# JeongsooP/RGB-no-more

Hardware: AMD Instinct MI355X
Metric: images/sec JPEG-Ti DCT 512x512 train step (higher is better)
Workload: dtype bf16

## Files before the change

rgb-no-more_amd/csrc/vit.hip:

```cpp
#include "common.h"
#include "../../include/rgbnm.h"

#define TRY(x)                 \
  do {                         \
    int rc__ = (x);            \
    if (rc__ != 0) return rc__; \
  } while (0)

static inline size_t max_sz(size_t a, size_t b) { return a > b ? a : b; }

#include <string.h>
#include <atomic>
#include <mutex>
#include <vector>
#include "internal.h"
namespace {
std::mutex g_trace_mu;
struct TraceRec { hipEvent_t a, b; int tag; double flops, bytes; };
std::vector<TraceRec> g_recs;
std::vector<hipEvent_t> g_event_pool;
hipEvent_t take_event() {
  if (!g_event_pool.empty()) { hipEvent_t e = g_event_pool.back(); g_event_pool.pop_back(); return e; }
  hipEvent_t e = nullptr;
  if (hipEventCreate(&e) != hipSuccess) return nullptr;
  return e;
}
struct Opt { const char* name; std::atomic<int> value; };
Opt g_opts[] = {{"nt_staged", 1}, {"tn_tr", 1}, {"tn_pipe", 1}, {"attn_v2", 1}, {"nt_wres", 1}, {"nt_kpipe", 1}, {"attn_persist", 1}, {"ln_fuse", 1}, {"tn_group", 2}, {"trace", 0}, {"tn_wgs", 512}, {"mlp_fuse", 1}, {"nt_cold", 0}, {"mlp_bwd", 1}, {"nt_small", 1}, {"mlp_dmast", 1}, {"gelu_table", 1}, {"ln_rows", 1}, {"kp8", 1}, {"win_xcd", 1}, {"kp_persist", 1}, {"fwd_chain", 1}, {"bwd_chain", 1}, {"tn_direct", 1}, {"tn_pack", 1}, {"tn_wide", 1}};
}

int rgbnm_trace_begin(int tag, double flops, double bytes, hipStream_t st) {
  int mask = 0;
  for (auto& o : g_opts) if (!strcmp(o.name, "trace")) mask = o.value.load(std::memory_order_relaxed);
  if (!((mask >> tag) & 1)) return -1;
  std::lock_guard<std::mutex> lk(g_trace_mu);
  TraceRec r;
  r.a = take_event();
  r.b = take_event();
  if (!r.a || !r.b) return -1;
  r.tag = tag; r.flops = flops; r.bytes = bytes;
  (void)hipEventRecord(r.a, st);
  g_recs.push_back(r);
  return (int)g_recs.size() - 1;
}
void rgbnm_trace_end(int slot, hipStream_t st) {
  if (slot < 0) return;
  std::lock_guard<std::mutex> lk(g_trace_mu);
  if (slot >= 0 && slot < (int)g_recs.size()) (void)hipEventRecord(g_recs[slot].b, st);
}

extern "C" {

int rgbnm_abi_version(void) { return RGBNM_ABI_VERSION; }

int rgbnm_set_option(const char* name, int value) {
  for (auto& o : g_opts)
    if (name && !strcmp(o.name, name)) { o.value.store(value, std::memory_order_relaxed); return RGBNM_OK; }
  return RGBNM_EINVAL;
}
int rgbnm_get_option(const char* name) {
  for (auto& o : g_opts)
    if (name && !strcmp(o.name, name)) return o.value.load(std::memory_order_relaxed);
  return -1;
}

int rgbnm_trace_reserve(int n_events) {
  if (n_events < 0 || n_events > (1 << 16)) return RGBNM_EINVAL;
  std::lock_guard<std::mutex> lk(g_trace_mu);
  while ((int)g_event_pool.size() < n_events) {
    hipEvent_t e = nullptr;
    if (hipEventCreate(&e) != hipSuccess) return RGBNM_ELAUNCH;
    g_event_pool.push_back(e);
  }
  return RGBNM_OK;
}

int rgbnm_trace_collect(int tag, double* ms_total, double* flops_total, double* bytes_total, int* count) {
  double ms = 0, fl = 0, by = 0;
  int n = 0;
  std::lock_guard<std::mutex> lk(g_trace_mu);
  std::vector<TraceRec> keep;
  for (auto& r : g_recs) {
    if (r.tag != tag) { keep.push_back(r); continue; }
    if (hipEventSynchronize(r.b) != hipSuccess) return RGBNM_ELAUNCH;
    float t = 0.f;
    if (hipEventElapsedTime(&t, r.a, r.b) != hipSuccess) return RGBNM_ELAUNCH;
    ms += t; fl += r.flops; by += r.bytes; ++n;
    g_event_pool.push_back(r.a);
    g_event_pool.push_back(r.b);
  }
  g_recs.swap(keep);
  if (ms_total) *ms_total = ms;
  if (flops_total) *flops_total = fl;
  if (bytes_total) *bytes_total = by;
  if (count) *count = n;
  return RGBNM_OK;
}

const char* rgbnm_strerror(int code) {
  switch (code) {
    case 0: return "ok";
    case RGBNM_EINVAL: return "invalid argument (null pointer, bad shape, alignment or dtype)";
    case RGBNM_ELAUNCH: return "HIP kernel launch failed";
    case RGBNM_EWORKSPACE: return "workspace too small";
    default: return "unknown rgbnm error";
  }
}

static bool fused_dx_lnbwd(int dt, const void* A, int lda, const void* Wt, int ldw, const void* x, const float* gamma,
                           const float* mean, const float* rstd, const void* dres, void* dx, float* dgamma,
                           float* dbeta, int M, int E, int K, void* ws, size_t ws_bytes, hipStream_t st) {
// ... 288 lines not shown
```

rgb-no-more_amd/csrc/vit_chain.hip:

```cpp
#include "common.h"
#include <string.h>
#include <type_traits>
#include "internal.h"
#include "../../include/rgbnm.h"

namespace {

typedef __attribute__((address_space(3))) void* lds_ptr;
typedef const __attribute__((address_space(1))) void* glb_ptr;
typedef unsigned int u32x2 __attribute__((ext_vector_type(2)));
typedef unsigned int u32x4 __attribute__((ext_vector_type(4)));
typedef bf16 bf16x2v __attribute__((ext_vector_type(2)));

constexpr int E = 192, HID = 768, HD = 64, HEADS = 3, NTOK = 196, NTILE = 7, NPAD = 224, INNER = HEADS * HD;
constexpr int NCW = 7, NTHREADS = 64 * (NCW + 1);
constexpr int ROWB = 128;
constexpr int SLOT = 24576;
constexpr int A_SLOT0 = 0;
constexpr int K_OFF = 3 * SLOT;
constexpr int ARR = NPAD * ROWB;
constexpr int V_OFF = K_OFF + ARR;
constexpr int STGA_OFF = V_OFF + ARR;
constexpr int STG_TILE = 32 * ROWB;
constexpr int MISC_OFF = STGA_OFF + 6 * STG_TILE + 4 * ROWB;
// ... 86 lines not shown
  template <typename F> static __device__ __forceinline__ void run(F&&) {}
};

__device__ __forceinline__ bf16x8 pack8(u32x2 lo, u32x2 hi) {
  u32x4 v = {lo[0], lo[1], hi[0], hi[1]};
  return __builtin_bit_cast(bf16x8, v);
}
template <int T>
__device__ __forceinline__ void tfrag4(unsigned a0, Frag<bf16> (&f)[4]) {
  u32x2 r0, r1, r2, r3, r4, r5, r6, r7;
  const unsigned a00 = a0, a01 = (a0 ^ 32u) + 1024u, a10 = a0 ^ 64u, a11 = (a0 ^ 96u) + 1024u;
  asm volatile(
      "ds_read_b64_tr_b16 %0, %8 offset:%12\n\t"
      "ds_read_b64_tr_b16 %1, %9 offset:%12\n\t"
      "ds_read_b64_tr_b16 %2, %10 offset:%12\n\t"
      "ds_read_b64_tr_b16 %3, %11 offset:%12\n\t"
      "ds_read_b64_tr_b16 %4, %8 offset:%13\n\t"
      "ds_read_b64_tr_b16 %5, %9 offset:%13\n\t"
      "ds_read_b64_tr_b16 %6, %10 offset:%13\n\t"
      "ds_read_b64_tr_b16 %7, %11 offset:%13\n\t"
      "s_waitcnt lgkmcnt(0)"
      : "=&v"(r0), "=&v"(r1), "=&v"(r2), "=&v"(r3), "=&v"(r4), "=&v"(r5), "=&v"(r6), "=&v"(r7)
      : "v"(a00), "v"(a01), "v"(a10), "v"(a11), "i"(T * 4096), "i"(T * 4096 + 2048)
      : "memory");
  __builtin_amdgcn_sched_barrier(0);
  f[0].v = pack8(r0, r1);
  f[1].v = pack8(r2, r3);
  f[2].v = pack8(r4, r5);
  f[3].v = pack8(r6, r7);
}
typedef bf16 bf16x4v __attribute__((ext_vector_type(4)));
typedef __attribute__((address_space(3))) bf16x4v* lds_b64_ptr;
__device__ __forceinline__ u32x2 tr_read(const unsigned char* smem, unsigned off) {
  return __builtin_bit_cast(u32x2, __builtin_amdgcn_ds_read_tr16_b64_v4bf16((lds_b64_ptr)(smem + off)));
}
template <int T>
__device__ __forceinline__ void tfrag4_b(const unsigned char* smem, unsigned a0, Frag<bf16> (&f)[4]) {
  const unsigned a00 = a0, a01 = (a0 ^ 32u) + 1024u, a10 = a0 ^ 64u, a11 = (a0 ^ 96u) + 1024u;
  f[0].v = pack8(tr_read(smem, a00 + T * 4096), tr_read(smem, a01 + T * 4096));
  f[1].v = pack8(tr_read(smem, a10 + T * 4096), tr_read(smem, a11 + T * 4096));
  f[2].v = pack8(tr_read(smem, a00 + T * 4096 + 2048), tr_read(smem, a01 + T * 4096 + 2048));
  f[3].v = pack8(tr_read(smem, a10 + T * 4096 + 2048), tr_read(smem, a11 + T * 4096 + 2048));
}
__device__ __forceinline__ Frag<bf16> pfrag(const float (&p)[16], int fi) {
  Frag<bf16> f;
#pragma unroll
  for (int j = 0; j < 8; ++j) f.v[j] = (bf16)p[fi * 8 + j];
  return f;
}

__device__ __forceinline__ unsigned opaque(unsigned v) {
  asm volatile("" : "+v"(v));
  return v;
}
__device__ __forceinline__ void wg_barrier() {
  asm volatile("" ::: "memory");
  __builtin_amdgcn_s_barrier();
  asm volatile("" ::: "memory");
}
template <int N> __device__ __forceinline__ void wait_vm() { asm volatile("s_waitcnt vmcnt(%0)" ::"n"(N) : "memory"); }
__device__ __forceinline__ void wait_lds() { asm volatile("s_waitcnt lgkmcnt(0)" ::: "memory"); }
#ifndef X_STORE
#define X_STORE 1
#endif
template <typename V, typename P>
__device__ __forceinline__ void gstore(P* ptr, const V& v) {
#if X_STORE == 1
  __builtin_nontemporal_store(v, reinterpret_cast<V*>(ptr));
#elif X_STORE == 2
  asm volatile("global_store_dwordx4 %0, %1, off sc1\n\ts_nop 2" ::"v"(reinterpret_cast<V*>(ptr)), "v"(v) : "memory");
#elif X_STORE == 3
  asm volatile("global_store_dwordx4 %0, %1, off sc0 sc1\n\ts_nop 2" ::"v"(reinterpret_cast<V*>(ptr)), "v"(v) : "memory");
#else
  *reinterpret_cast<V*>(ptr) = v;
#endif
}

#ifdef X_LDSWAIT
__device__ __forceinline__ void own_tile_fence() { wait_lds(); }
#else
__device__ __forceinline__ void own_tile_fence() { asm volatile("" ::: "memory"); }
#endif

template <int NKB>
__device__ __forceinline__ void dma_linear(const unsigned char* src, unsigned char* dst, int lane) {
#pragma unroll
  for (int i = 0; i < NKB; ++i)
    __builtin_amdgcn_global_load_lds((glb_ptr)(src + i * 1024 + lane * 16), (lds_ptr)(dst + i * 1024), 16, 0, 0);
}
__device__ __forceinline__ void dma_f32x192(const float* src, unsigned char* dst, int lane) {
#pragma unroll
  for (int i = 0; i < 3; ++i)
    __builtin_amdgcn_global_load_lds((glb_ptr)(src + 64 * i + lane), (lds_ptr)(dst + 256 * i), 4, 0, 0);
}

struct Rows { u32x4 v[12]; };
__device__ __forceinline__ float bf_lo(unsigned u) { return __builtin_bit_cast(float, u << 16); }
__device__ __forceinline__ float bf_hi(unsigned u) { return __builtin_bit_cast(float, u & 0xffff0000u); }
__device__ __forceinline__ unsigned pack2(float a, float b) {
  const bf16x2v v = {(bf16)a, (bf16)b};
  unsigned r = __builtin_bit_cast(unsigned, v);
  asm volatile("" : "+v"(r));
  return r;
}
__device__ __forceinline__ bf16x8 as_bf16x8(u32x4 v) { return __builtin_bit_cast(bf16x8, v); }

__device__ __forceinline__ void ln_stats(const Rows& x, float& mu, float& rs, float eps) {
  float s0 = 0.f, s1 = 0.f;
#pragma unroll
  for (int c = 0; c < 12; ++c)
#pragma unroll
    for (int d = 0; d < 4; ++d) {
      const unsigned u = opaque(x.v[c][d]);
      s0 += bf_lo(u);
      s1 += bf_hi(u);
    }
  float s = s0 + s1;
  s += __shfl_xor(s, 32, 64);
  mu = s * (1.f / E);
  float q0 = 0.f, q1 = 0.f;
#pragma unroll
  for (int c = 0; c < 12; ++c)
#pragma unroll
    for (int d = 0; d < 4; ++d) {
      const unsigned u = opaque(x.v[c][d]);
      const float d0 = bf_lo(u) - mu, d1 = bf_hi(u) - mu;
      q0 = __builtin_fmaf(d0, d0, q0);
      q1 = __builtin_fmaf(d1, d1, q1);
    }
  float q = q0 + q1;
  q += __shfl_xor(q, 32, 64);
  rs = rsqrtf(__builtin_fmaf(q, 1.f / E, eps));
}
__device__ __forceinline__ void ln_apply(const Rows& x, float mu, float rs, const float* gb, int g, Rows& y) {
#ifdef X_NOLN
#pragma unroll
  for (int c = 0; c < 12; ++c) y.v[c] = x.v[c];
  return;
#endif
#pragma unroll
  for (int c = 0; c < 12; ++c) {
    const float* gp = gb + 16 * c + 8 * g;
    const f32x4 g0 = *reinterpret_cast<const f32x4*>(gp), g1 = *reinterpret_cast<const f32x4*>(gp + 4);
    const f32x4 b0 = *reinterpret_cast<const f32x4*>(gp + E), b1 = *reinterpret_cast<const f32x4*>(gp + E + 4);
#pragma unroll
    for (int d = 0; d < 4; ++d) {
      const float gm0 = d < 2 ? g0[2 * d] : g1[2 * d - 4], gm1 = d < 2 ? g0[2 * d + 1] : g1[2 * d - 3];
      const float bt0 = d < 2 ? b0[2 * d] : b1[2 * d - 4], bt1 = d < 2 ? b0[2 * d + 1] : b1[2 * d - 3];
      const unsigned u = opaque(x.v[c][d]);
      y.v[c][d] = pack2(__builtin_fmaf((bf_lo(u) - mu) * rs, gm0, bt0), __builtin_fmaf((bf_hi(u) - mu) * rs, gm1, bt1));
    }
    if (c & 1) __builtin_amdgcn_sched_barrier(0);
  }
}

__device__ __forceinline__ void tile_out(unsigned char* smem, unsigned stg, const u32x4& p0, const u32x4& p1, const u32x4& p2,
                                         const u32x4& p3, bf16* dst, int ld, int live) {
  const int ln = lane_id_here();
  const unsigned wo = stg + (unsigned)((ln & 31) * ROWB + (((ln >> 5) ^ (ln & 7)) << 4));
  if ((ln & 31) < live) {
    *reinterpret_cast<u32x4*>(smem + wo) = p0;
    *reinterpret_cast<u32x4*>(smem + (wo ^ 32u)) = p1;
    *reinterpret_cast<u32x4*>(smem + (wo ^ 64u)) = p2;
    *reinterpret_cast<u32x4*>(smem + (wo ^ 96u)) = p3;
  }
  own_tile_fence();
  const int rl = ln >> 3, seg = ln & 7;
  const unsigned ro = stg + (unsigned)(rl * ROWB + ((seg ^ rl) << 4));
  bf16* gp = dst + (size_t)rl * ld + seg * 8;
  u32x4 v[4];
#pragma unroll
  for (int i = 0; i < 4; ++i) v[i] = *reinterpret_cast<const u32x4*>(smem + ro + i * 8 * ROWB);
#ifndef X_NOSAVE
  if (live == 32) {
#pragma unroll
    for (int i = 0; i < 4; ++i) gstore(gp + (size_t)i * 8 * ld, v[i]);
  } else {
#pragma unroll
    for (int i = 0; i < 4; ++i)
      if (i * 8 + rl < live) gstore(gp + (size_t)i * 8 * ld, v[i]);
  }
#endif
  own_tile_fence();
}
__device__ __forceinline__ void rows_out(unsigned char* smem, unsigned stg, const Rows& x, bf16* dst, int live) {
#pragma unroll
  for (int t = 0; t < 3; ++t) {
    tile_out(smem, stg, x.v[4 * t], x.v[4 * t + 1], x.v[4 * t + 2], x.v[4 * t + 3], dst + 64 * t, E, live);
    __builtin_amdgcn_sched_barrier(0);
  }
}

__device__ __forceinline__ void gemm_k192(f32x16& acc, const unsigned char* sW, int ht, const Rows& x, const Geo& L) {
  int wbase = L.l31 * (E * 2) + ((L.g ^ L.fl) << 4) + ht * 32 * (E * 2);
  asm volatile("" : "+v"(wbase));
  Frag<bf16> fb;
#pragma unroll
  for (int c = 0; c < 12; ++c) {
    Frag<bf16> fx;
#ifdef X_HALFW
    if ((c & 1) == 0)
#endif
    fb.v = *reinterpret_cast<const bf16x8*>(sW + ((wbase ^ ((c % 4) << 5)) + 128 * (c / 4)));
    fx.v = as_bf16x8(x.v[c]);
    mma(acc, fb, fx);
  }
}

template <int DEPTH>
__device__ __forceinline__ void gemm_k192x2(f32x16& a0, f32x16& a1, const unsigned char* sW, const Rows& x, const Geo& L) {
  int wb0 = L.l31 * (E * 2) + ((L.g ^ L.fl) << 4);
  asm volatile("" : "+v"(wb0));
  const int wb1 = wb0 + 32 * (E * 2);
  Frag<bf16> fb[24];
#pragma unroll
  for (int i = 0; i < 24; ++i) {
    const int c = i >> 1;
    fb[i].v = *reinterpret_cast<const bf16x8*>(sW + ((((i & 1) ? wb1 : wb0) ^ ((c % 4) << 5)) + 128 * (c / 4)));
  }
#pragma unroll
  for (int i = 0; i < 24; ++i) {
    Frag<bf16> fx;
    fx.v = as_bf16x8(x.v[i >> 1]);
    mma((i & 1) ? a1 : a0, fb[i], fx);
  }
  __builtin_amdgcn_sched_group_barrier(0x100, DEPTH, 0);
#pragma unroll
  for (int i = 0; i < 24 - DEPTH; ++i) {
    __builtin_amdgcn_sched_group_barrier(0x008, 1, 0);
    __builtin_amdgcn_sched_group_barrier(0x100, 1, 0);
  }
#pragma unroll
  for (int i = 0; i < DEPTH; ++i) __builtin_amdgcn_sched_group_barrier(0x008, 1, 0);
}

#ifdef CHAIN_PROF
#ifndef CHAIN_PROF_BLK
#define CHAIN_PROF_BLK 1
#endif
__device__ unsigned long long g_chain_prof[8 * 8 * 128];
#define CP(i)                                                                                          \
  do {                                                                                                 \
    if (ib == CHAIN_PROF_BLK && blockIdx.x < 8) {                                                      \
      const unsigned long long t_ = __builtin_amdgcn_s_memtime();                                      \
      if ((threadIdx.x & 63) == 0) g_chain_prof[(blockIdx.x * 8 + (threadIdx.x >> 6)) * 128 + (i)] = t_; \
    }                                                                                                  \
  } while (0)
#define CP_RT(i)                                                                                       \
  do {                                                                                                 \
    if (blockIdx.x < 8 && (threadIdx.x & 63) == 0)                                                     \
      g_chain_prof[(blockIdx.x * 8 + (threadIdx.x >> 6)) * 128 + (i)] = __builtin_amdgcn_s_memrealtime(); \
  } while (0)
#else
#define CP(i) do {} while (0)
#define CP_RT(i) do {} while (0)
#endif
#define BAR(s) do { CP(2 * (s)); wg_barrier(); CP(2 * (s) + 1); } while (0)
// ... 324 lines not shown
          pf = pfrag(pr, 1);
          mma(o[0], vv[2], pf);
          mma(o[1], vv[3], pf);
        });
#else
        {
          Frag<bf16> kc[4], kn[4];
#pragma unroll
          for (int c = 0; c < 4; ++c) kc[c].v = *reinterpret_cast<const bf16x8*>(Ks + (rb ^ (unsigned)(c << 5)));
          __builtin_amdgcn_sched_barrier(0);
          TileLoop<NTILE>::run([&](auto tc) {
            constexpr int t = decltype(tc)::value;
            f32x16 acc;
#pragma unroll
            for (int r = 0; r < 16; ++r) acc[r] = 0.f;
#pragma unroll
            for (int c = 0; c < 4; ++c) mma(acc, kc[c], qf[c]);
            Frag<bf16> vv[4];
            tfrag4_b<t>(smem, vt, vv);
            if (t + 1 < NTILE) {
#pragma unroll
              for (int c = 0; c < 4; ++c)
                kn[c].v = *reinterpret_cast<const bf16x8*>(Ks + (rb ^ (unsigned)(c << 5)) + (t + 1) * 32 * ROWB);
            }
            float pr[16];
#pragma unroll
            for (int r = 0; r < 16; ++r) {
#ifdef X_NOEXP
              pr[r] = fmaf(acc[r], c2, -mc2);
#else
              pr[r] = __builtin_amdgcn_exp2f(fmaf(acc[r], c2, -mc2));
#endif
              if (t * 32 + 32 > NTOK && t * 32 + acc_row(r, L.lane) >= NTOK) pr[r] = 0.f;
              sum += pr[r];
            }
            Frag<bf16> pf = pfrag(pr, 0);
            mma(o[0], vv[0], pf);
            mma(o[1], vv[1], pf);
            pf = pfrag(pr, 1);
            mma(o[0], vv[2], pf);
            mma(o[1], vv[3], pf);
            __builtin_amdgcn_sched_group_barrier(0x008, 4, 0);
            if (t + 1 < NTILE) __builtin_amdgcn_sched_group_barrier(0x100, 12, 0);
            else __builtin_amdgcn_sched_group_barrier(0x100, 8, 0);
            __builtin_amdgcn_sched_group_barrier(0x008, 4, 0);
            __builtin_amdgcn_sched_barrier(0);
#pragma unroll
            for (int c = 0; c < 4; ++c) kc[c] = kn[c];
          });
        }
#endif
        sum += __shfl_xor(sum, 32, 64);
        const float inv = 1.f / sum;
        if (L.g == 0 && L.l31 < live) b.lse[((size_t)img * HEADS + h) * NTOK + row0 + L.l31] = mx * p.scale + __logf(sum);
        u32x4 op[4];
#pragma unroll
        for (int dt = 0; dt < 2; ++dt)
#pragma unroll
          for (int hs = 0; hs < 2; ++hs) {
#pragma unroll
            for (int d = 0; d < 4; ++d) op[2 * dt + hs][d] = pack2(o[dt][8 * hs + 2 * d] * inv, o[dt][8 * hs + 2 * d + 1] * inv);
            of[h][2 * dt + hs].v = as_bf16x8(op[2 * dt + hs]);
          }
        {
          const int ln = lane_id_here();
          const unsigned wo = stg + (unsigned)((ln & 31) * ROWB + ((ln & 7) << 4) + (ln >> 5) * 8);
          if ((ln & 31) < live)
#pragma unroll
          for (int dt = 0; dt < 2; ++dt)
#pragma unroll
            for (int rq = 0; rq < 4; ++rq) {
              const u32x4 src = op[2 * dt + (rq >> 1)];
              const u32x2 q2 = {src[2 * (rq & 1)], src[2 * (rq & 1) + 1]};
              *reinterpret_cast<u32x2*>(smem + (wo ^ (unsigned)((dt * 4 + rq) << 4))) = q2;
            }
          own_tile_fence();
          const int rl = ln >> 3, seg = ln & 7;
          const unsigned ro = stg + (unsigned)(rl * ROWB + ((seg ^ rl) << 4));
          bf16* dst = b.attn + (grow0 + rl) * INNER + h * HD + seg * 8;
          u32x4 v[4];
#pragma unroll
          for (int i = 0; i < 4; ++i) v[i] = *reinterpret_cast<const u32x4*>(smem + ro + i * 8 * ROWB);
#ifndef X_NOSAVE
          if (live == 32) {
#pragma unroll
            for (int i = 0; i < 4; ++i) gstore(dst + (size_t)i * 8 * INNER, v[i]);
          } else {
#pragma unroll
            for (int i = 0; i < 4; ++i)
              if (i * 8 + rl < live) gstore(dst + (size_t)i * 8 * INNER, v[i]);
          }
#endif
          own_tile_fence();
        }
      }
    }
    const Geo L = fresh_geo();
    f32x16 accp[6];
#pragma unroll
    for (int bt = 0; bt < 6; ++bt)
#pragma unroll
      for (int r = 0; r < 16; ++r) accp[bt][r] = 0.f;
#pragma unroll
    for (int h = 0; h < HEADS; ++h) {
      BAR(12 + h);
      const unsigned wo = opaque((unsigned)(A_SLOT0 + h * SLOT + L.l31 * ROWB + ((L.g ^ L.fl) << 4)));
#pragma unroll
      for (int s = 0; s < 4; ++s) {
        Frag<bf16> fw[6];
#pragma unroll
        for (int bt = 0; bt < 6; ++bt)
#ifdef X_HALFW
          if (bt & 1) fw[bt].v = fw[bt - 1].v; else
#endif
          fw[bt].v = *reinterpret_cast<const bf16x8*>(smem + (wo ^ (unsigned)(s << 5)) + bt * 32 * ROWB);
#pragma unroll
        for (int bt = 0; bt < 6; ++bt) mma(accp[bt], fw[bt], of[h][s]);
      }
#ifndef X_NOPIPE
      __builtin_amdgcn_sched_group_barrier(0x100, PIPE_P, 0);
#pragma unroll
      for (int i = 0; i < 24 - PIPE_P; ++i) {
        __builtin_amdgcn_sched_group_barrier(0x008, 1, 0);
        __builtin_amdgcn_sched_group_barrier(0x100, 1, 0);
      }
#pragma unroll
      for (int i = 0; i < PIPE_P; ++i) __builtin_amdgcn_sched_group_barrier(0x008, 1, 0);
      __builtin_amdgcn_sched_barrier(0);
#endif
    }
    BAR(15);
    float mu2, rs2;
    {
#pragma unroll
      for (int c = 0; c < 12; ++c) {
        const float* bp = bprj + 16 * c + 8 * L.g;
        const f32x4 b0 = *reinterpret_cast<const f32x4*>(bp), b1 = *reinterpret_cast<const f32x4*>(bp + 4);
#pragma unroll
        for (int d = 0; d < 4; ++d) {
          const unsigned u = opaque(xr.v[c][d]);
          xr.v[c][d] = pack2(accp[c >> 1][8 * (c & 1) + 2 * d] + (d < 2 ? b0[2 * d] : b1[2 * d - 4]) + bf_lo(u),
                             accp[c >> 1][8 * (c & 1) + 2 * d + 1] + (d < 2 ? b0[2 * d + 1] : b1[2 * d - 3]) + bf_hi(u));
        }
        if (c & 1) __builtin_amdgcn_sched_barrier(0);
      }
      __builtin_amdgcn_sched_barrier(0);
      ln_stats(xr, mu2, rs2, p.eps);
      __builtin_amdgcn_sched_barrier(0);
      rows_out(smem, stg, xr, b.x_mid + grow0 * E, live);
      __builtin_amdgcn_sched_barrier(0);
      if (L.g == 0 && L.l31 < live) {
        b.mean2[grow0 + L.l31] = mu2;
        b.rstd2[grow0 + L.l31] = rs2;
      }
    }
    Rows fa;
    __builtin_amdgcn_sched_barrier(0);
    ln_apply(xr, mu2, rs2, ln2p, L.g, fa);
    __builtin_amdgcn_sched_barrier(0);
    rows_out(smem, stg, fa, b.xn2 + grow0 * E, live);
    __builtin_amdgcn_sched_barrier(0);

    f32x16 acc2[6];
#pragma unroll
    for (int c = 0; c < 12; ++c)
#pragma unroll
      for (int d = 0; d < 4; ++d) {
// ... 317 lines not shown
```

rgb-no-more_amd/csrc/vit_chain_bwd.hip:

```cpp
#include "common.h"
#include <string.h>
#include <type_traits>
#include "internal.h"
#include "ln_bwd_rows.h"
#include "../../include/rgbnm.h"

namespace {

typedef __attribute__((address_space(3))) void* lds_ptr;
typedef const __attribute__((address_space(1))) void* glb_ptr;
typedef unsigned int u32x2 __attribute__((ext_vector_type(2)));
typedef unsigned int u32x4 __attribute__((ext_vector_type(4)));
typedef bf16 bf16x2v __attribute__((ext_vector_type(2)));

constexpr int E = 192, HID = 768, HD = 64, HEADS = 3, NTOK = 196, NTILE = 7, NPAD = 224, INNER = HEADS * HD, LDQ = 3 * INNER;
constexpr int NCW = 7, NTHREADS = 64 * (NCW + 1), CTHREADS = 64 * NCW, BM = 32 * NCW;
constexpr int ROWB = 128, ARR = NPAD * ROWB, SLOT = 24576, STAGE = 2 * SLOT, CH = 64, NCHUNK = HID / CH;
constexpr int CP = E + 4;
constexpr int SMEM = 163840;
#ifndef PIPE_P
#define PIPE_P 6
#endif
#ifndef PIPE_M1
#define PIPE_M1 5
#endif
#ifndef PIPE_X
#define PIPE_X 7
#endif
constexpr int M_STG = 2 * STAGE;
constexpr int TILE = 32 * ROWB;
typedef rgbnm::LnBwdRows<CTHREADS, BM> LnBwd;
constexpr int RED_OFF = (BM * CP * 2 + 1023) / 1024 * 1024;
static_assert(RED_OFF + LnBwd::RED_BYTES <= 132096, "LDS");
constexpr int P_SLOT0 = 132096, P_SLOT1 = 0, P_TILES = 98304;
static_assert(P_SLOT0 + SLOT <= SMEM && P_TILES + NCW * TILE <= P_SLOT0, "LDS");
constexpr int A_Q = 0, A_K = ARR, A_V = 2 * ARR, A_G = 3 * ARR, A_L2 = 4 * ARR, A_D = A_L2 + NPAD * 4, A_STG = A_D + NPAD * 4;
constexpr int STG_PITCH = 144, STG_WAVE = 32 * STG_PITCH;
constexpr int A_SIDE = A_STG + NCW * STG_WAVE;
static_assert(A_SIDE + NCW * 1024 <= SMEM, "LDS");
constexpr int X_SLOT0 = A_K, X_SLOT1 = A_K + SLOT, X_SLOT2 = 0, X_TILES = A_K + 2 * SLOT, X_TSET = NCW * TILE;
static_assert(X_SLOT1 + SLOT <= X_TILES && X_TILES + 3 * X_TSET <= SMEM && SLOT <= A_K, "LDS");

struct BwdBlk {
  const bf16* wimg;
  const float *ln1_g, *ln2_g;
  const bf16* x_in; const float *mean1, *rstd1;
  const bf16* qkv; const float* lse; const bf16* attn; const bf16* x_mid; const float *mean2, *rstd2; const bf16* gp;
  const bf16* dy;
  bf16* du; bf16* dx_mid; bf16* dqkv; bf16* dx;
  float *part2, *part1;
};
static_assert(sizeof(BwdBlk) == sizeof(rgbnm_chain_bwd_block), "rgbnm_chain_bwd_block layout");
constexpr int MAX_DEPTH = 12;
struct BwdArgs {
  BwdBlk blk[MAX_DEPTH]; bf16* dattn;
  int depth, nimg;
  float scale;
};

__device__ __forceinline__ int fswz(int row) {
  return (((row >> 1) & 1) << 2) | ((row >> 2) & 1) | (((row >> 3) & 1) << 1);
}
struct Geo {
  int lane, l31, g, fl;
  unsigned tr0;
};
__device__ __forceinline__ Geo make_geo() {
  Geo L;
  L.lane = threadIdx.x & 63;
  L.l31 = L.lane & 31;
  L.g = L.lane >> 5;
  L.fl = fswz(L.l31);
  const int k = (L.lane >> 2) & 3, G1 = (L.lane >> 4) & 1, l3 = L.lane & 3;
  const int pc = (2 * G1 + (l3 >> 1)) ^ (((k >> 1) << 2) | L.g);
  L.tr0 = (unsigned)((4 * L.g + k) * ROWB + pc * 16 + 8 * (l3 & 1));
  return L;
}
__device__ __forceinline__ Geo fresh_geo() {
  Geo L;
  L.lane = lane_id_here();
  L.l31 = L.lane & 31;
  L.g = L.lane >> 5;
  L.fl = fswz(L.l31);
  const int k = (L.lane >> 2) & 3, G1 = (L.lane >> 4) & 1, l3 = L.lane & 3;
  const int pc = (2 * G1 + (l3 >> 1)) ^ (((k >> 1) << 2) | L.g);
  L.tr0 = (unsigned)((4 * L.g + k) * ROWB + pc * 16 + 8 * (l3 & 1));
  return L;
}
template <int T> struct TileLoop {
  template <typename F> static __device__ __forceinline__ void run(F&& f) {
    TileLoop<T - 1>::run(f);
    f(std::integral_constant<int, T - 1>{});
  }
};
template <> struct TileLoop<0> {
  template <typename F> static __device__ __forceinline__ void run(F&&) {}
};
__device__ __forceinline__ bf16x8 pack8(u32x2 lo, u32x2 hi) {
  u32x4 v = {lo[0], lo[1], hi[0], hi[1]};
  return __builtin_bit_cast(bf16x8, v);
}
template <int T>
__device__ __forceinline__ void tfrag4(unsigned a0, Frag<bf16> (&f)[4]) {
  u32x2 r0, r1, r2, r3, r4, r5, r6, r7;
  const unsigned a00 = a0, a01 = (a0 ^ 32u) + 1024u, a10 = a0 ^ 64u, a11 = (a0 ^ 96u) + 1024u;
  asm volatile(
      "ds_read_b64_tr_b16 %0, %8 offset:%12\n\t"
      "ds_read_b64_tr_b16 %1, %9 offset:%12\n\t"
      "ds_read_b64_tr_b16 %2, %10 offset:%12\n\t"
      "ds_read_b64_tr_b16 %3, %11 offset:%12\n\t"
      "ds_read_b64_tr_b16 %4, %8 offset:%13\n\t"
      "ds_read_b64_tr_b16 %5, %9 offset:%13\n\t"
      "ds_read_b64_tr_b16 %6, %10 offset:%13\n\t"
// ... 230 lines not shown
      const int r = i * 8 + rl;
      v[wv][i] = PRIVATE ? *reinterpret_cast<const u32x4*>(src + wv * STG_WAVE + r * STG_PITCH + seg * 16)
                         : *reinterpret_cast<const u32x4*>(src + (wv * 32 + r) * ROWB + ((seg ^ (r & 7)) << 4));
    }
}
__device__ __forceinline__ void tiles_write(const u32x4 (&v)[NTILE][4], bf16* __restrict__ g0, size_t ld, int lane) {
  const int rl = lane >> 3, seg = lane & 7;
#pragma unroll
  for (int wv = 0; wv < NTILE; ++wv)
#pragma unroll
    for (int i = 0; i < 4; ++i) {
      const int row = wv * 32 + i * 8 + rl;
      if (row < NTOK) gstore<(XB_NT & 2) != 0>(g0 + (size_t)row * ld + seg * 8, v[wv][i]);
    }
}

#ifdef CHAINB_PROF
__device__ unsigned long long g_chainb_prof[8 * 8 * 128];
#define CP_(i)                                                                                          \
  do {                                                                                                  \
    if (ib == CHAINB_PROF_BLK && blockIdx.x < 8) {                                                      \
      const unsigned long long t_ = __builtin_amdgcn_s_memtime();                                       \
      if ((threadIdx.x & 63) == 0) g_chainb_prof[(blockIdx.x * 8 + (threadIdx.x >> 6)) * 128 + (i)] = t_; \
    }                                                                                                   \
  } while (0)
#ifndef CHAINB_PROF_BLK
#define CHAINB_PROF_BLK 6
#endif
#else
#define CP_(i) do {} while (0)
#endif
#define BAR(s) do { CP_(2 * (s)); wg_barrier(); CP_(2 * (s) + 1); } while (0)
constexpr int B_M0 = 0;
constexpr int B_E2 = 12;
constexpr int B_P = 19;
constexpr int B_A = 24;
constexpr int B_X = 37;
constexpr int B_E1 = 46;
constexpr int B_END = 53;

__device__ __forceinline__ void ln_bwd_request(LnBwd& lnb, const bf16* X, const float* mean, const float* rstd, const bf16* R, int img,
                                               int w) {
  const int tid = w * 64 + lane_id_here();
  lnb.request_x(X, E, mean, rstd, img * NTOK, NTOK, tid);
  lnb.request_res(R, E, img * NTOK, NTOK, tid);
}
template <int B0>
__device__ __forceinline__ void ln_bwd_epilogue(unsigned char* smem, const f32x16 (&acc)[6], const bf16* X, const float* mean,
                                                const float* rstd, const bf16* R, const float* gamma, bf16* DX,
                                                float* part, int img, int w, int ib) {
  const int lane_ = lane_id_here();
  const int tid = w * 64 + lane_, rloc = w * 32 + (lane_ & 31), g = lane_ >> 5;
  LnBwd lnb;
  lnb.request_x(X, E, mean, rstd, img * NTOK, NTOK, tid);
  lnb.request_res(R, E, img * NTOK, NTOK, tid);
  wait_lds();
  BAR(B0);
  bf16* Cs = reinterpret_cast<bf16*>(smem);
#pragma unroll
  for (int b = 0; b < 6; ++b)
#pragma unroll
    for (int q = 0; q < 4; ++q) {
      const int nl = 32 * b + 8 * q + 4 * g;
      const f32x4 v = {acc[b][4 * q + 0], acc[b][4 * q + 1], acc[b][4 * q + 2], acc[b][4 * q + 3]};
      store4<bf16>(Cs + rloc * CP + nl, v);
    }
  wait_lds();
  BAR(B0 + 1);
  lnb.run<true>(Cs, CP, DX, E, gamma, true, part, img, reinterpret_cast<float*>(smem + RED_OFF), img * NTOK, NTOK, tid, Cs,
          [&](int k) { if (k == 0) BAR(B0 + 2); else if (k == 1) BAR(B0 + 3); else if (k == 2) BAR(B0 + 4); else BAR(B0 + 5); });
  wait_lds();
  BAR(B0 + 6);
}
__device__ __forceinline__ void read_own_rows(const unsigned char* smem, int w, Rows& x) {
  const int lane_ = lane_id_here();
  const unsigned char* rp = smem + (w * 32 + (lane_ & 31)) * (CP * 2) + 16 * (lane_ >> 5);
#pragma unroll
  for (int c = 0; c < 12; ++c) {
    const u32x2 lo = *reinterpret_cast<const u32x2*>(rp + 32 * c), hi = *reinterpret_cast<const u32x2*>(rp + 32 * c + 8);
    x.v[c] = u32x4{lo[0], lo[1], hi[0], hi[1]};
  }
}

__global__ __launch_bounds__(NTHREADS) void vit_chain_bwd_kernel(BwdArgs p) {
  extern __shared__ __attribute__((aligned(16))) unsigned char smem[];
  const int img = blockIdx.x;
  if (img >= p.nimg) return;
  const int w = __builtin_amdgcn_readfirstlane(threadIdx.x >> 6);
  const int depth = p.depth;

  if (w == NCW) {
#ifdef X_DMAPRIO
    __builtin_amdgcn_s_setprio(X_DMAPRIO);
#endif
    const int lane = threadIdx.x & 63;
    for (int ib = depth - 1; ib >= 0; --ib) {
      const BwdBlk& b = p.blk[ib];
      const unsigned char* wimg = reinterpret_cast<const unsigned char*>(b.wimg);
      dma_linear<48>(wimg, smem, lane);
      for (int c = 0; c < NCHUNK; ++c) {
        wait_vm<0>();
        BAR(B_M0 + c);
        if (c + 1 < NCHUNK) dma_linear<48>(wimg + (size_t)(c + 1) * STAGE, smem + ((c + 1) & 1) * STAGE, lane);
      }
      BAR(B_E2);
      dma_linear<24>(wimg + (size_t)NCHUNK * STAGE, smem + P_SLOT0, lane);
#pragma unroll
      for (int k = 1; k < 7; ++k) BAR(B_E2 + k);
      const bf16* qkv0 = b.qkv + (size_t)img * NTOK * LDQ;
      const bf16* do0 = p.dattn + (size_t)img * NTOK * INNER;
      bf16* dq0 = b.dqkv + (size_t)img * NTOK * LDQ;
      const unsigned char* stg0 = smem + A_STG;
      auto issue_kv = [&](int h) {
        dma_matrix_all(qkv0 + INNER + h * HD, LDQ, smem + A_K, lane);
        dma_matrix_all(qkv0 + 2 * INNER + h * HD, LDQ, smem + A_V, lane);
      };
      auto issue_q = [&](int h) { dma_matrix_all(qkv0 + h * HD, LDQ, smem + A_Q, lane); };
      auto issue_g = [&](int h) { dma_matrix_all(do0 + h * HD, INNER, smem + A_G, lane); };
      const unsigned char* xw = wimg + (size_t)NCHUNK * STAGE + 3 * SLOT;
      auto issue_xt = [&](int j) { dma_row_tiles(dq0 + j * 64, LDQ, smem + X_TILES + (j % 3) * X_TSET, lane); };
      wait_vm<0>();
      BAR(B_P);
      BAR(B_P + 1);
      dma_linear<24>(wimg + (size_t)NCHUNK * STAGE + SLOT, smem + P_SLOT1, lane);
      issue_kv(0);
      wait_vm<56>(); BAR(B_P + 2);
      dma_linear<24>(wimg + (size_t)NCHUNK * STAGE + 2 * SLOT, smem + P_SLOT0, lane);
      wait_vm<0>(); BAR(B_P + 3);
      issue_q(0);
      BAR(B_P + 4);
      {
        issue_g(0);
        wait_vm<0>();
        BAR(B_A);
        for (int h = 0; h < HEADS; ++h) {
          bf16* g0 = dq0 + h * HD;
          wait_vm<0>();
          BAR(B_A + 1 + 4 * h);
          u32x4 tq[NTILE][4];
          tiles_read<true>(stg0, lane, tq);
          wait_lds();
          BAR(B_A + 2 + 4 * h);
          tiles_write(tq, g0, LDQ, lane);
          if (h + 1 < HEADS) issue_kv(h + 1);
          else {
            dma_linear<24>(xw, smem + X_SLOT0, lane);
            dma_linear<24>(xw + SLOT, smem + X_SLOT1, lane);
          }
          wait_vm<0>();
          BAR(B_A + 3 + 4 * h);
          tiles_read<true>(stg0, lane, tq);
          wait_lds();
          BAR(B_A + 4 + 4 * h);
          tiles_write(tq, g0 + INNER, LDQ, lane);
          tiles_read<false>(smem + A_G, lane, tq);
          wait_lds();
          if (h + 1 < HEADS) {
            issue_q(h + 1);
            issue_g(h + 1);
          } else {
            issue_xt(0);
          }
          tiles_write(tq, g0 + 2 * INNER, LDQ, lane);
        }
      }
      for (int j = 0; j < 9; ++j) {
        if (j == 0) wait_vm<28>();
        else if (j + 1 < 9) wait_vm<52>();
        else wait_vm<0>();
        BAR(B_X + j);
        if (j == 0) {
          issue_xt(1);
          dma_linear<24>(xw + 2 * SLOT, smem + X_SLOT2, lane);
          issue_xt(2);
        }
        if (j + 2 < 9 && j >= 1) {
          dma_linear<24>(xw + (size_t)(j + 2) * SLOT, smem + ((j + 2) % 3 == 0 ? X_SLOT0 : ((j + 2) % 3 == 1 ? X_SLOT1 : X_SLOT2)), lane);
          issue_xt(j + 2);
        }
      }
#pragma unroll
      for (int k = 0; k < 7; ++k) BAR(B_E1 + k);
      BAR(B_END);
    }
    return;
  }

#if defined(X_PRIO) && X_PRIO == 1
  if (w >= 4) __builtin_amdgcn_s_setprio(1);
#elif defined(X_PRIO) && X_PRIO == 2
  if (w < 4) __builtin_amdgcn_s_setprio(1);
#endif
  const int row0 = 32 * w;
  const int live = NTOK - row0 < 32 ? NTOK - row0 : 32;
  const size_t grow0 = (size_t)img * NTOK + row0;
  const float LOG2E = 1.4426950408889634f;
  const float c2 = p.scale * LOG2E;

  Rows dyf;
  {
    const int lane_ = lane_id_here();
    const int rloc = row0 + (lane_ & 31), tok = rloc < NTOK ? rloc : NTOK - 1;
    const bf16* yrow = p.blk[depth - 1].dy + ((size_t)img * NTOK + tok) * E + 8 * (lane_ >> 5);
#pragma unroll
    for (int c = 0; c < 12; ++c) dyf.v[c] = *reinterpret_cast<const u32x4*>(yrow + 16 * c);
  }

  for (int ib = depth - 1; ib >= 0; --ib) {
    const BwdBlk& b = p.blk[ib];
    f32x16 acc2[6];
#pragma unroll
    for (int bt = 0; bt < 6; ++bt)
#pragma unroll
      for (int r = 0; r < 16; ++r) acc2[bt][r] = 0.f;
    {
      const Geo L = fresh_geo();
      const int fl = L.fl;
      const int woff0 = L.l31 * (E * 2) + ((L.g ^ fl) << 4);
      const unsigned stg = (unsigned)(M_STG + w * 2 * TILE);
      bf16x8 gpraw[4];
      auto load_gp = [&](int chunk) {
        const int ln = lane_id_here();
#pragma unroll
        for (int i = 0; i < 4; ++i) {
          const int idx = ln + 64 * i, row = idx >> 3, vec = idx & 7;
          int rr = row0 + row;
          rr = rr < NTOK ? rr : NTOK - 1;
          const bf16x8* gsrc = reinterpret_cast<const bf16x8*>(b.gp + ((size_t)img * NTOK + rr) * HID + chunk * CH + vec * 8);
          gpraw[i] = (XB_NTLD & 1) ? __builtin_nontemporal_load(gsrc) : *gsrc;
        }
      };
      load_gp(0);
      for (int chunk = 0; chunk < NCHUNK; ++chunk) {
        {
          const int ln = lane_id_here();
#pragma unroll
          for (int i = 0; i < 4; ++i) {
            const int idx = ln + 64 * i, row = idx >> 3, vec = idx & 7;
            *reinterpret_cast<bf16x8*>(smem + stg + row * ROWB + ((vec ^ (row & 7)) << 4)) = gpraw[i];
          }
        }
        if (chunk + 1 < NCHUNK) load_gp(chunk + 1);
        wait_lds();
        BAR(B_M0 + chunk);
        const unsigned st_off = (unsigned)((chunk & 1) * STAGE);
        const unsigned char* sW1 = smem + st_off;
        const unsigned w2o = opaque(st_off + (unsigned)(SLOT + L.l31 * ROWB + ((L.g ^ fl) << 4)));
        const unsigned two = opaque(stg + (unsigned)(L.l31 * ROWB + ((L.g ^ (L.l31 & 7)) << 4)));
#pragma unroll
        for (int ht = 0; ht < 2; ++ht) {
          f32x16 a1;
#pragma unroll
          for (int r = 0; r < 16; ++r) a1[r] = 0.f;
          int wbase = woff0 + ht * 32 * (E * 2);
          asm volatile("" : "+v"(wbase));
#ifdef X_NOPIPE
#pragma unroll
          for (int c = 0; c < 12; ++c) {
            Frag<bf16> fb, fx;
            fb.v = *reinterpret_cast<const bf16x8*>(sW1 + ((wbase ^ ((c % 4) << 5)) + 128 * (c / 4)));
            fx.v = as_bf16x8(dyf.v[c]);
            mma(a1, fb, fx);
          }
#else
          {
            Frag<bf16> fb[12];
#pragma unroll
            for (int c = 0; c < 12; ++c)
              fb[c].v = *reinterpret_cast<const bf16x8*>(sW1 + ((wbase ^ ((c % 4) << 5)) + 128 * (c / 4)));
#pragma unroll
            for (int c = 0; c < 12; ++c) {
              Frag<bf16> fx;
              fx.v = as_bf16x8(dyf.v[c]);
              mma(a1, fb[c], fx);
            }
            __builtin_amdgcn_sched_group_barrier(0x100, PIPE_M1, 0);
#pragma unroll
            for (int i = 0; i < 12 - PIPE_M1; ++i) {
              __builtin_amdgcn_sched_group_barrier(0x008, 1, 0);
              __builtin_amdgcn_sched_group_barrier(0x100, 1, 0);
            }
#pragma unroll
            for (int i = 0; i < PIPE_M1; ++i) __builtin_amdgcn_sched_group_barrier(0x008, 1, 0);
            __builtin_amdgcn_sched_barrier(0);
          }
          Frag<bf16> fw2[12];
#pragma unroll
          for (int bt = 0; bt < 6; ++bt)
            fw2[bt].v = *reinterpret_cast<const bf16x8*>(smem + (w2o ^ (unsigned)((2 * ht) << 5)) + bt * 32 * ROWB);
          __builtin_amdgcn_sched_barrier(0);
#endif
          Frag<bf16> pg[2];
#pragma unroll
          for (int hs = 0; hs < 2; ++hs) {
            const unsigned to = two ^ (unsigned)((2 * ht + hs) << 5);
            const bf16x8 gpv = *reinterpret_cast<const bf16x8*>(smem + to);
            bf16x8 dv;
#pragma unroll
            for (int j = 0; j < 8; ++j) dv[j] = (bf16)((float)(bf16)a1[8 * hs + j] * (float)gpv[j]);
            pg[hs].v = dv;
            *reinterpret_cast<bf16x8*>(smem + to + TILE) = dv;
          }
#ifdef X_NOPIPE
#pragma unroll
          for (int hs = 0; hs < 2; ++hs) {
            const int s = 2 * ht + hs;
            Frag<bf16> fw[6];
#pragma unroll
            for (int bt = 0; bt < 6; ++bt)
              fw[bt].v = *reinterpret_cast<const bf16x8*>(smem + (w2o ^ (unsigned)(s << 5)) + bt * 32 * ROWB);
#pragma unroll
            for (int bt = 0; bt < 6; ++bt) mma(acc2[bt], fw[bt], pg[hs]);
          }
#else
          __builtin_amdgcn_sched_barrier(0);
#pragma unroll
          for (int bt = 0; bt < 6; ++bt)
            fw2[6 + bt].v = *reinterpret_cast<const bf16x8*>(smem + (w2o ^ (unsigned)((2 * ht + 1) << 5)) + bt * 32 * ROWB);
#pragma unroll
          for (int bt = 0; bt < 6; ++bt) mma(acc2[bt], fw2[bt], pg[0]);
#pragma unroll
          for (int bt = 0; bt < 6; ++bt) mma(acc2[bt], fw2[6 + bt], pg[1]);
#pragma unroll
          for (int i = 0; i < 6; ++i) {
            __builtin_amdgcn_sched_group_barrier(0x008, 1, 0);
            __builtin_amdgcn_sched_group_barrier(0x100, 1, 0);
          }
          __builtin_amdgcn_sched_group_barrier(0x008, 6, 0);
          __builtin_amdgcn_sched_barrier(0);
#endif
        }
        own_tile_fence();
        const int ln = lane_id_here();
        bf16x8 dv0[4];
#pragma unroll
        for (int i = 0; i < 4; ++i) {
          const int idx = ln + 64 * i, row = idx >> 3, vec = idx & 7;
          dv0[i] = *reinterpret_cast<const bf16x8*>(smem + stg + TILE + row * ROWB + ((vec ^ (row & 7)) << 4));
        }
        if (live == 32) {
#pragma unroll
          for (int i = 0; i < 4; ++i) {
            const int idx = ln + 64 * i, row = idx >> 3, vec = idx & 7;
            gstore<(XB_NT & 1) != 0>(b.du + (grow0 + row) * HID + chunk * CH + vec * 8, dv0[i]);
          }
        } else {
#pragma unroll
          for (int i = 0; i < 4; ++i) {
            const int idx = ln + 64 * i, row = idx >> 3, vec = idx & 7;
            if (row < live) gstore<(XB_NT & 1) != 0>(b.du + (grow0 + row) * HID + chunk * CH + vec * 8, dv0[i]);
          }
        }
      }
    }
    ln_bwd_epilogue<B_E2>(smem, acc2, b.x_mid, b.mean2, b.rstd2, b.dy, b.ln2_g, b.dx_mid, b.part2, img, w, ib);
    {
      const Geo L = fresh_geo();
      Rows dxf;
      read_own_rows(smem, w, dxf);
      wait_lds();
      BAR(B_P);
      const unsigned stg = (unsigned)(P_TILES + w * TILE);
#pragma unroll
      for (int h = 0; h < HEADS; ++h) {
        BAR(B_P + 1 + h);
        const unsigned char* sW = smem + (h == 1 ? P_SLOT1 : P_SLOT0);
        f32x16 acc[2];
#pragma unroll
        for (int ht = 0; ht < 2; ++ht)
#pragma unroll
          for (int r = 0; r < 16; ++r) acc[ht][r] = 0.f;
#ifdef X_NOPIPE
        gemm_k192(acc[0], sW, 0, dxf, L);
        gemm_k192(acc[1], sW, 1, dxf, L);
#else
        gemm_k192x2<PIPE_P>(acc[0], acc[1], sW, dxf, L);
#endif
        u32x4 pc[4];
#pragma unroll
        for (int ht = 0; ht < 2; ++ht)
#pragma unroll
          for (int hs = 0; hs < 2; ++hs)
#pragma unroll
            for (int d = 0; d < 4; ++d) pc[2 * ht + hs][d] = pack2(acc[ht][8 * hs + 2 * d], acc[ht][8 * hs + 2 * d + 1]);
        tile_out(smem, stg, pc[0], pc[1], pc[2], pc[3], p.dattn + grow0 * INNER + h * HD, INNER, live);
      }
      asm volatile("s_waitcnt vmcnt(0)" ::: "memory");
      BAR(B_P + 4);
    }
    {
      unsigned char* Qs = smem + A_Q;
      unsigned char* Ks = smem + A_K;
      unsigned char* Vs = smem + A_V;
      unsigned char* Gs = smem + A_G;
      float* L2_s = reinterpret_cast<float*>(smem + A_L2);
      float* D_s = reinterpret_cast<float*>(smem + A_D);
      unsigned char* stg = smem + A_STG + w * STG_WAVE;
      const Geo L = fresh_geo();
      const int fl = L.fl;
      const unsigned rb0 = (unsigned)(L.l31 * ROWB + ((L.g ^ fl) << 4));
      const int row = row0 + L.l31;
      u32x4 qraw[4], graw[4], oraw[4];
      float lq = 0.f;
      const bf16* qkv0 = b.qkv + (size_t)img * NTOK * LDQ;
      const bf16* do0 = p.dattn + (size_t)img * NTOK * INNER;
      const bf16* o0 = b.attn + (size_t)img * NTOK * INNER;
      auto load_own_g = [&](int h) {
        const int lane_ = lane_id_here();
        const int seg = lane_ & 7;
#pragma unroll
        for (int i = 0; i < 4; ++i) {
          int r = row0 + i * 8 + (lane_ >> 3);
          r = r < NTOK ? r : NTOK - 1;
          graw[i] = *reinterpret_cast<const u32x4*>(do0 + (size_t)r * INNER + h * HD + seg * 8);
        }
      };
      unsigned char* qside = smem + A_SIDE + w * 1024;
      auto load_own_q = [&](int h) {
        const int lane_ = lane_id_here();
        const int seg = lane_ & 7;
#pragma unroll
        for (int i = 0; i < 4; ++i) {
          int r = row0 + i * 8 + (lane_ >> 3);
          r = r < NTOK ? r : NTOK - 1;
          const bf16* src = qkv0 + (size_t)r * LDQ + h * HD + seg * 8;
          if (i == 0) __builtin_amdgcn_global_load_lds((glb_ptr)src, (lds_ptr)qside, 16, 0, 0);
          else qraw[i] = *reinterpret_cast<const u32x4*>(src);
        }
      };
      auto load_own_o = [&](int h) {
        const int lane_ = lane_id_here();
        const int seg = lane_ & 7;
#pragma unroll
// ... 128 lines not shown
            mma(dv[1], gg[1], f);
            f = pfrag(pp, 1);
            mma(dv[0], gg[2], f);
            mma(dv[1], gg[3], f);
            tfrag4<t>(qt_, gg);
            f = pfrag(ds, 0);
            mma(dk[0], gg[0], f);
            mma(dk[1], gg[1], f);
            f = pfrag(ds, 1);
            mma(dk[0], gg[2], f);
            mma(dk[1], gg[3], f);
          });
          if (more) load_own_g(h + 1);
          tile_park_private(stg, dk, p.scale, L);
          if (more) load_own_q(h + 1);
          wait_lds();
          BAR(B_A + 3 + 4 * h);
          tile_park_rows(Gs, w, dv, 1.0f);
        }
        if (more) load_own_o(h + 1);
        wait_lds();
        BAR(B_A + 4 + 4 * h);
      }
    }
    f32x16 accx[6];
#pragma unroll
    for (int bt = 0; bt < 6; ++bt)
#pragma unroll
      for (int r = 0; r < 16; ++r) accx[bt][r] = 0.f;
    for (int j = 0; j < 9; ++j) {
      BAR(B_X + j);
      const Geo L = fresh_geo();
      const int fl = L.fl;
      const int set = j % 3;
      const unsigned wo = opaque((unsigned)((set == 0 ? X_SLOT0 : (set == 1 ? X_SLOT1 : X_SLOT2)) + L.l31 * ROWB + ((L.g ^ fl) << 4)));
      const unsigned to = opaque((unsigned)(X_TILES + set * X_TSET + w * TILE + L.l31 * ROWB + ((L.g ^ (L.l31 & 7)) << 4)));
#pragma unroll
      for (int s = 0; s < 4; ++s) {
        Frag<bf16> fx, fw[6];
        fx.v = *reinterpret_cast<const bf16x8*>(smem + (to ^ (unsigned)(s << 5)));
#pragma unroll
        for (int bt = 0; bt < 6; ++bt)
          fw[bt].v = *reinterpret_cast<const bf16x8*>(smem + (wo ^ (unsigned)(s << 5)) + bt * 32 * ROWB);
#pragma unroll
        for (int bt = 0; bt < 6; ++bt) mma(accx[bt], fw[bt], fx);
      }
#ifndef X_NOPIPE
      __builtin_amdgcn_sched_group_barrier(0x100, PIPE_X, 0);
#pragma unroll
      for (int i = 0; i < 24; ++i) {
        __builtin_amdgcn_sched_group_barrier(0x008, 1, 0);
        if (i < 28 - PIPE_X) __builtin_amdgcn_sched_group_barrier(0x100, 1, 0);
      }
      __builtin_amdgcn_sched_barrier(0);
#endif
    }
    ln_bwd_epilogue<B_E1>(smem, accx, b.x_in, b.mean1, b.rstd1, b.dx_mid, b.ln1_g, b.dx, b.part1, img, w, ib);
    read_own_rows(smem, w, dyf);
    wait_lds();
    BAR(B_END);
  }
}

}

#ifdef CHAINB_PROF
extern "C" int rgbnm_chainb_prof_read(unsigned long long* host_out) {
  return hipMemcpyFromSymbol(host_out, HIP_SYMBOL(g_chainb_prof), sizeof(unsigned long long) * 8 * 8 * 128) == hipSuccess ? 0 : -1;
}
#endif

extern "C" {

size_t rgbnm_chain_bwd_block_bytes(void) { return sizeof(BwdBlk); }

int rgbnm_vit_chain_bwd(const rgbnm_vit_cfg* c, const rgbnm_chain_bwd_block* blocks, int depth, void* dattn, void* stream) {
  if (!c || !blocks || !dattn || depth <= 0) return RGBNM_EINVAL;
  if (c->dtype != RGBNM_DT_BF16 || c->E != E || c->heads != HEADS || c->N != NTOK || c->B < 1 || depth > MAX_DEPTH) return 1;
  BwdArgs p;
  memcpy(p.blk, blocks, sizeof(BwdBlk) * depth);
  p.dattn = (bf16*)dattn; p.depth = depth; p.nimg = c->B; p.scale = c->attn_scale;
  static DevOnce attr;
  if (attr.need()) {
    if (hipFuncSetAttribute((const void*)vit_chain_bwd_kernel, hipFuncAttributeMaxDynamicSharedMemorySize, SMEM) != hipSuccess)
      return RGBNM_ELAUNCH;
    attr.done();
  }
  const double tok = (double)c->B * NTOK;
  const double flops = depth * tok * 2.0 * (2.0 * E * HID + INNER * E + 3.0 * INNER * E + 4.0 * NTOK * INNER);
  const double bytes = depth * (tok * ((2.0 * HID + 5.0 * E + 2.0 * 3.0 * INNER) * 2.0 + 4 * 4 + HEADS * 4) + 36.0 * SLOT) + tok * E * 2.0;
  const int slot = rgbnm_trace_begin(TR_CHAIN_BWD, flops, bytes, (hipStream_t)stream);
  hipLaunchKernelGGL(vit_chain_bwd_kernel, dim3(c->B), dim3(NTHREADS), SMEM, (hipStream_t)stream, p);
  rgbnm_trace_end(slot, (hipStream_t)stream);
  LAUNCH_CHECK();
  return RGBNM_OK;
}

}
```

Before: 66140.

## Hand off young-warp du tile stores to partner warps in chain backward

Adds a templated HAND variant of the chained backward kernel, enabled by a new default-on option. Warps 4-6 no longer write their du tile to global memory on every chunk. On odd chunks they stage it in a spare LDS buffer, and partner warps 0-2 store the previous chunk's tile for them, which spreads global stores more evenly across warps. The change also adds debug-only macros that drop stores, plus extra LDS usage and cross-warp timing dependencies that rely on existing barriers for correctness.

```diff
diff --git a/rgb-no-more_amd/csrc/vit.hip b/rgb-no-more_amd/csrc/vit.hip
--- a/rgb-no-more_amd/csrc/vit.hip
+++ b/rgb-no-more_amd/csrc/vit.hip
@@ -26,7 +26,7 @@
   return e;
 }
 struct Opt { const char* name; std::atomic<int> value; };
-Opt g_opts[] = {{"nt_staged", 1}, {"tn_tr", 1}, {"tn_pipe", 1}, {"attn_v2", 1}, {"nt_wres", 1}, {"nt_kpipe", 1}, {"attn_persist", 1}, {"ln_fuse", 1}, {"tn_group", 2}, {"trace", 0}, {"tn_wgs", 512}, {"mlp_fuse", 1}, {"nt_cold", 0}, {"mlp_bwd", 1}, {"nt_small", 1}, {"mlp_dmast", 1}, {"gelu_table", 1}, {"ln_rows", 1}, {"kp8", 1}, {"win_xcd", 1}, {"kp_persist", 1}, {"fwd_chain", 1}, {"bwd_chain", 1}, {"tn_direct", 1}, {"tn_pack", 1}, {"tn_wide", 1}};
+Opt g_opts[] = {{"nt_staged", 1}, {"tn_tr", 1}, {"tn_pipe", 1}, {"attn_v2", 1}, {"nt_wres", 1}, {"nt_kpipe", 1}, {"attn_persist", 1}, {"ln_fuse", 1}, {"tn_group", 2}, {"trace", 0}, {"tn_wgs", 512}, {"mlp_fuse", 1}, {"nt_cold", 0}, {"mlp_bwd", 1}, {"nt_small", 1}, {"mlp_dmast", 1}, {"gelu_table", 1}, {"ln_rows", 1}, {"kp8", 1}, {"win_xcd", 1}, {"kp_persist", 1}, {"fwd_chain", 1}, {"bwd_chain", 1}, {"chain_hand", 1}, {"tn_direct", 1}, {"tn_pack", 1}, {"tn_wide", 1}};
 }
 
 int rgbnm_trace_begin(int tag, double flops, double bytes, hipStream_t st) {
diff --git a/rgb-no-more_amd/csrc/vit_chain.hip b/rgb-no-more_amd/csrc/vit_chain.hip
--- a/rgb-no-more_amd/csrc/vit_chain.hip
+++ b/rgb-no-more_amd/csrc/vit_chain.hip
@@ -192,6 +192,12 @@
 __device__ __forceinline__ void own_tile_fence() { asm volatile("" ::: "memory"); }
 #endif
 
+#ifdef X_NOSAVE_YOUNG
+__device__ __forceinline__ bool drop_row_stores() { return __builtin_amdgcn_readfirstlane(threadIdx.x >> 6) >= 4; }
+#else
+__device__ __forceinline__ bool drop_row_stores() { return false; }
+#endif
+
 template <int NKB>
 __device__ __forceinline__ void dma_linear(const unsigned char* src, unsigned char* dst, int lane) {
 #pragma unroll
@@ -282,7 +288,8 @@
 #pragma unroll
   for (int i = 0; i < 4; ++i) v[i] = *reinterpret_cast<const u32x4*>(smem + ro + i * 8 * ROWB);
 #ifndef X_NOSAVE
-  if (live == 32) {
+  if (drop_row_stores()) {
+  } else if (live == 32) {
 #pragma unroll
     for (int i = 0; i < 4; ++i) gstore(gp + (size_t)i * 8 * ld, v[i]);
   } else {
@@ -773,7 +780,8 @@
 #pragma unroll
           for (int i = 0; i < 4; ++i) v[i] = *reinterpret_cast<const u32x4*>(smem + ro + i * 8 * ROWB);
 #ifndef X_NOSAVE
-          if (live == 32) {
+          if (drop_row_stores()) {
+          } else if (live == 32) {
 #pragma unroll
             for (int i = 0; i < 4; ++i) gstore(dst + (size_t)i * 8 * INNER, v[i]);
           } else {
diff --git a/rgb-no-more_amd/csrc/vit_chain_bwd.hip b/rgb-no-more_amd/csrc/vit_chain_bwd.hip
--- a/rgb-no-more_amd/csrc/vit_chain_bwd.hip
+++ b/rgb-no-more_amd/csrc/vit_chain_bwd.hip
@@ -29,6 +29,8 @@
 #endif
 constexpr int M_STG = 2 * STAGE;
 constexpr int TILE = 32 * ROWB;
+constexpr int M_DU2 = M_STG + NCW * 2 * TILE;
+static_assert(M_DU2 + 2 * TILE <= SMEM, "LDS");
 typedef rgbnm::LnBwdRows<CTHREADS, BM> LnBwd;
 constexpr int RED_OFF = (BM * CP * 2 + 1023) / 1024 * 1024;
 static_assert(RED_OFF + LnBwd::RED_BYTES <= 132096, "LDS");
@@ -425,6 +427,7 @@
   }
 }
 
+template <bool HAND>
 __global__ __launch_bounds__(NTHREADS) void vit_chain_bwd_kernel(BwdArgs p) {
   extern __shared__ __attribute__((aligned(16))) unsigned char smem[];
   const int img = blockIdx.x;
@@ -561,6 +564,8 @@
       const int fl = L.fl;
       const int woff0 = L.l31 * (E * 2) + ((L.g ^ fl) << 4);
       const unsigned stg = (unsigned)(M_STG + w * 2 * TILE);
+      const bool young = HAND && w >= 4;
+      const bool partner = HAND && w < NCW - 4;
       bf16x8 gpraw[4];
       auto load_gp = [&](int chunk) {
         const int ln = lane_id_here();
@@ -590,6 +595,7 @@
         const unsigned char* sW1 = smem + st_off;
         const unsigned w2o = opaque(st_off + (unsigned)(SLOT + L.l31 * ROWB + ((L.g ^ fl) << 4)));
         const unsigned two = opaque(stg + (unsigned)(L.l31 * ROWB + ((L.g ^ (L.l31 & 7)) << 4)));
+        const unsigned dut = !(young && (chunk & 1)) ? stg + TILE : (unsigned)(w < 6 ? M_DU2 + (w - 4) * TILE : stg + TILE + 8 * ROWB);
 #pragma unroll
         for (int ht = 0; ht < 2; ++ht) {
           f32x16 a1;
@@ -642,7 +648,7 @@
 #pragma unroll
             for (int j = 0; j < 8; ++j) dv[j] = (bf16)((float)(bf16)a1[8 * hs + j] * (float)gpv[j]);
             pg[hs].v = dv;
-            *reinterpret_cast<bf16x8*>(smem + to + TILE) = dv;
+            if (!HAND || L.l31 < live) *reinterpret_cast<bf16x8*>(smem + to + (dut - stg)) = dv;
           }
 #ifdef X_NOPIPE
 #pragma unroll
@@ -675,23 +681,57 @@
         }
         own_tile_fence();
         const int ln = lane_id_here();
-        bf16x8 dv0[4];
-#pragma unroll
-        for (int i = 0; i < 4; ++i) {
-          const int idx = ln + 64 * i, row = idx >> 3, vec = idx & 7;
-          dv0[i] = *reinterpret_cast<const bf16x8*>(smem + stg + TILE + row * ROWB + ((vec ^ (row & 7)) << 4));
-        }
-        if (live == 32) {
+        if (!young || chunk == NCHUNK - 1) {
+          bf16x8 dv0[4];
 #pragma unroll
           for (int i = 0; i < 4; ++i) {
             const int idx = ln + 64 * i, row = idx >> 3, vec = idx & 7;
-            gstore<(XB_NT & 1) != 0>(b.du + (grow0 + row) * HID + chunk * CH + vec * 8, dv0[i]);
-          }
-        } else {
-#pragma unroll
-          for (int i = 0; i < 4; ++i) {
-            const int idx = ln + 64 * i, row = idx >> 3, vec = idx & 7;
-            if (row < live) gstore<(XB_NT & 1) != 0>(b.du + (grow0 + row) * HID + chunk * CH + vec * 8, dv0[i]);
+            dv0[i] = *reinterpret_cast<const bf16x8*>(smem + dut + row * ROWB + ((vec ^ (row & 7)) << 4));
+          }
+#ifdef XB_NOSAVE_YOUNG
+          if (w >= 4) {
+          } else
+#endif
+          if (live == 32) {
+#pragma unroll
+            for (int i = 0; i < 4; ++i) {
+              const int idx = ln + 64 * i, row = idx >> 3, vec = idx & 7;
+              gstore<(XB_NT & 1) != 0>(b.du + (grow0 + row) * HID + chunk * CH + vec * 8, dv0[i]);
+            }
+          } else {
+#pragma unroll
+            for (int i = 0; i < 4; ++i) {
+              const int idx = ln + 64 * i, row = idx >> 3, vec = idx & 7;
+              if (row < live) gstore<(XB_NT & 1) != 0>(b.du + (grow0 + row) * HID + chunk * CH + vec * 8, dv0[i]);
+            }
+          }
+        }
+        if (partner && chunk > 0) {
+          const unsigned pt = (unsigned)((chunk & 1) ? M_STG + (w + 4) * 2 * TILE + TILE
+                                                     : (w < 2 ? M_DU2 + w * TILE : M_STG + (w + 4) * 2 * TILE + TILE + 8 * ROWB));
+          bf16* hdst = b.du + (grow0 + 4 * 32) * HID + (chunk - 1) * CH;
+          if (w < 2) {
+            bf16x8 hv[4];
+#pragma unroll
+            for (int i = 0; i < 4; ++i) {
+              const int idx = ln + 64 * i, row = idx >> 3, vec = idx & 7;
+              hv[i] = *reinterpret_cast<const bf16x8*>(smem + pt + row * ROWB + ((vec ^ (row & 7)) << 4));
+            }
+#ifndef XB_NOSAVE_YOUNG
+#pragma unroll
+            for (int i = 0; i < 4; ++i) {
+              const int idx = ln + 64 * i, row = idx >> 3, vec = idx & 7;
+              gstore<(XB_NT & 1) != 0>(hdst + (size_t)row * HID + vec * 8, hv[i]);
+            }
+#endif
+          } else {
+            const int row = ln >> 3, vec = ln & 7;
+            if (row < NTOK - 6 * 32) {
+              const bf16x8 hv = *reinterpret_cast<const bf16x8*>(smem + pt + row * ROWB + ((vec ^ (row & 7)) << 4));
+#ifndef XB_NOSAVE_YOUNG
+              gstore<(XB_NT & 1) != 0>(hdst + (size_t)row * HID + vec * 8, hv);
+#endif
+            }
           }
         }
       }
@@ -986,7 +1026,8 @@
   p.dattn = (bf16*)dattn; p.depth = depth; p.nimg = c->B; p.scale = c->attn_scale;
   static DevOnce attr;
   if (attr.need()) {
-    if (hipFuncSetAttribute((const void*)vit_chain_bwd_kernel, hipFuncAttributeMaxDynamicSharedMemorySize, SMEM) != hipSuccess)
+    if (hipFuncSetAttribute((const void*)vit_chain_bwd_kernel<false>, hipFuncAttributeMaxDynamicSharedMemorySize, SMEM) != hipSuccess ||
+        hipFuncSetAttribute((const void*)vit_chain_bwd_kernel<true>, hipFuncAttributeMaxDynamicSharedMemorySize, SMEM) != hipSuccess)
       return RGBNM_ELAUNCH;
     attr.done();
   }
@@ -994,7 +1035,10 @@
   const double flops = depth * tok * 2.0 * (2.0 * E * HID + INNER * E + 3.0 * INNER * E + 4.0 * NTOK * INNER);
   const double bytes = depth * (tok * ((2.0 * HID + 5.0 * E + 2.0 * 3.0 * INNER) * 2.0 + 4 * 4 + HEADS * 4) + 36.0 * SLOT) + tok * E * 2.0;
   const int slot = rgbnm_trace_begin(TR_CHAIN_BWD, flops, bytes, (hipStream_t)stream);
-  hipLaunchKernelGGL(vit_chain_bwd_kernel, dim3(c->B), dim3(NTHREADS), SMEM, (hipStream_t)stream, p);
+  if (rgbnm_get_option("chain_hand"))
+    hipLaunchKernelGGL(vit_chain_bwd_kernel<true>, dim3(c->B), dim3(NTHREADS), SMEM, (hipStream_t)stream, p);
+  else
+    hipLaunchKernelGGL(vit_chain_bwd_kernel<false>, dim3(c->B), dim3(NTHREADS), SMEM, (hipStream_t)stream, p);
   rgbnm_trace_end(slot, (hipStream_t)stream);
   LAUNCH_CHECK();
   return RGBNM_OK;
```

New measurement: 66250, median of 6. About the same (+0.2%).
